# SEAME-pt/Team02-ObjectDetection

Hardware: AMD Instinct MI355X
Metric: images/sec fwd+bwd MobileNetV2UNet 256x512 bs=32/GPU (higher is better)
Workload: dtype f32; 1 GPU; MobileNetV2UNet 10-class fwd+bwd+Adam, 256x512, bs=32/GPU (BASELINE configs[1]); model=MobileNetV2UNet, global_batch=32, parallelism=dp1, collectives=RCCL (torch.distributed nccl), optimizer=seg_amd.Adam (HIP, one launch)

## Files before the change

### include/segamd.h

```cpp
#ifndef SEGAMD_H
#define SEGAMD_H
#include <hip/hip_runtime.h>
#include <stdint.h>
#ifdef __cplusplus
extern "C" {
#endif



int seg_conv_igemm(const float* in, long ldin, int N, int H, int W, int Cin,
                   const float* wk, int ldk, const float* bias,
                   float* out, long ldout, int Ho, int Wo, int Cout,
                   int ks, int stride, int pad,
                   const float* add, long ldadd, float* stat, hipStream_t stream);
int seg_conv_igemm_act(const float* in, long ldin, int N, int H, int W, int Cin,
                       const float* wk, int ldk, const float* bias,
                       float* out, long ldout, int Ho, int Wo, int Cout,
                       int ks, int stride, int pad,
                       const float* add, long ldadd, float* stat, int act, float* work, int splits,
                       hipStream_t stream);
int seg_conv_igemm_bf16(const float* in, long ldin, int N, int H, int W, int Cin,
                        const float* wk, int ldk, const float* bias,
                        float* out, long ldout, int Ho, int Wo, int Cout,
                        int ks, int stride, int pad,
                        const float* add, long ldadd, float* stat, int act, float* work, int splits,
                        hipStream_t stream);
int seg_conv_igemm_f16(const float* in, long ldin, int N, int H, int W, int Cin,
                       const float* wk, int ldk, const float* bias,
                       float* out, long ldout, int Ho, int Wo, int Cout,
                       int ks, int stride, int pad,
                       const float* add, long ldadd, float* stat, int act, float* work, int splits,
                       hipStream_t stream);
int seg_conv_pw_row_tiles(long M);
int seg_conv_pw(const float* in, long ldin, long M, int K, const float* wk, int ldk, const float* bias,
                float* out, long ldout, int N, const float* add, long ldadd, float* stat,
                const float* in_scale, const float* in_shift, int in_act, hipStream_t stream);
int seg_conv_igemm_splits(long M, int Cout, int Cin, int ks);
int seg_conv_igemm_tiles(long M, int Cout);
int seg_conv_igemm_plan_b1(long M, int Cout, int Cin, int ks, int* out);
int seg_conv_igemm_act_ic(const float* in, long ldin, int N, int H, int W, int Cin, const float* wk, int ldk,
                          const float* bias, float* out, long ldout, int Ho, int Wo, int Cout, int ks, int stride,
                          int pad, const float* add, long ldadd, int act, float* work, int splits, int tile, unsigned* cnt,
                          hipStream_t stream);
int seg_conv_igemm_bf16_ic(const float* in, long ldin, int N, int H, int W, int Cin, const float* wk, int ldk,
                           const float* bias, float* out, long ldout, int Ho, int Wo, int Cout, int ks, int stride,
                           int pad, const float* add, long ldadd, int act, float* work, int splits, int tile, unsigned* cnt,
                           hipStream_t stream);
int seg_conv_igemm_f16_ic(const float* in, long ldin, int N, int H, int W, int Cin, const float* wk, int ldk,
                          const float* bias, float* out, long ldout, int Ho, int Wo, int Cout, int ks, int stride,
                          int pad, const float* add, long ldadd, int act, float* work, int splits, int tile, unsigned* cnt,
                          hipStream_t stream);

int seg_conv_igemm_bnout_ok(long M, int Cout, int bf16);
int seg_conv_igemm_bnout(const float* in, long ldin, int N, int H, int W, int Cin, const float* wk, int ldk,
                         float* out, long ldout, int Cout, int ks, const float* add, long ldadd,
                         const float* by, long ldby, const float* bscale, const float* bshift,
                         const float* bmean, int bact, float* bpart, hipStream_t stream);

int seg_igemm_force_tile(int t);
int seg_conv_igemm_tile(long M, int Cout);
int seg_conv_igemm_row_tiles(long M, int Cout, int* tile_rows);

int seg_pack_conv_weight(const float* w, float* wk, int Cout, int Cin, int ks, int ldk,
                         int mode, int kin_pad, hipStream_t stream);

int seg_conv_wgrad_splits(long M, int Cout, int Cin, int ks);
int seg_conv_wgrad_splits_bf16(long M, int Cout, int Cin, int ks);
int seg_conv_wgrad(const float* dy, long lddy, const float* x, long ldx,
                   int N, int H, int W, int Cin, int Ho, int Wo, int Cout,
                   int ks, int stride, int pad, float* part, int splits, hipStream_t stream);

int seg_conv_wgrad_bf16(const float* dy, long lddy, const float* x, long ldx,
                        int N, int H, int W, int Cin, int Ho, int Wo, int Cout,
                        int ks, int stride, int pad, float* part, int splits, hipStream_t stream);

int seg_conv_igemm_xf(const float* in, long ldin, int N, int H, int W, int Cin,
                      const float* wk, int ldk, const float* bias,
                      float* out, long ldout, int Ho, int Wo, int Cout,
                      int ks, int stride, int pad,
                      const float* add, long ldadd, float* stat, const float* in_scale, const float* in_shift,
                      int in_act, hipStream_t stream);
int seg_conv_igemm_bf16_xf(const float* in, long ldin, int N, int H, int W, int Cin,
                           const float* wk, int ldk, const float* bias,
                           float* out, long ldout, int Ho, int Wo, int Cout,
                           int ks, int stride, int pad,
                           const float* add, long ldadd, float* stat, const float* in_scale, const float* in_shift,
                           int in_act, hipStream_t stream);
int seg_conv_wgrad_xf(const float* dy, long lddy, const float* x, long ldx,
                      int N, int H, int W, int Cin, int Ho, int Wo, int Cout,
                      int ks, int stride, int pad, float* part, int splits,
                      const float* in_scale, const float* in_shift, int in_act, hipStream_t stream);
int seg_conv_wgrad_bf16_xf(const float* dy, long lddy, const float* x, long ldx,
                           int N, int H, int W, int Cin, int Ho, int Wo, int Cout,
                           int ks, int stride, int pad, float* part, int splits,
                           const float* in_scale, const float* in_shift, int in_act, hipStream_t stream);

int seg_conv_wgrad_reduce(const float* part, int splits, float* dw, int Cout, int Cin, int ks,
                          int mode, int accumulate, hipStream_t stream);

int seg_conv_wino_pick(int N, int H, int W, int Cin, int Cout);
int seg_conv_wino_tile_rows(void);
int seg_conv_wino_row_tiles(int N, int H, int W);
int seg_conv_wino(const float* in, long ldin, int N, int H, int W, int Cin, const float* wk, int ldk,
                  const float* bias, float* out, long ldout, int Cout, const float* add, long ldadd,
                  float* stat, float* work, hipStream_t stream);
int seg_conv_wino_fused(const float* in, long ldin, int N, int H, int W, int Cin, const float* wk, int ldk,
                        const float* bias, float* out, long ldout, int Cout, const float* add, long ldadd, float* stat,
                        hipStream_t stream);
int seg_conv_wino_fused_ok(int N, int H, int W, long ldin);
int seg_conv_wino_wgrad_pick(int N, int H, int W, int Cin, int Cout);
int seg_conv_wino_wgrad_splits(int N, int H, int W, int Cin, int Cout);
int seg_conv_wino_wgrad(const float* dy, long lddy, const float* x, long ldx, int N, int H, int W, int Cin,
                        int Cout, float* part, int splits, hipStream_t stream);
int seg_conv_wino_wgrad16_splits(int N, int H, int W, int Cin, int Cout);
int seg_conv_wino_wgrad16(const float* dy, long lddy, const float* x, long ldx, int N, int H, int W, int Cin,
                          int Cout, float* part, int splits, hipStream_t stream);
int seg_conv_wino_wgrad_reduce(float* part, int splits, float* dw, int Cout, int Cin, int Cin_pad,
                               int accumulate, hipStream_t stream);

int seg_conv_halo_ok(int N, int H, int W, int Cin, int Cout);
int seg_conv_halo_pick(int N, int H, int W, int Cin, int Cout);
int seg_conv_halo_row_tiles(int N, int H, int W);
int seg_conv_halo(const float* in, long ldin, int N, int H, int W, int Cin, const float* wk, int ldk,
                  const float* bias, float* out, long ldout, int Cout, const float* add, long ldadd,
                  float* stat, hipStream_t stream);

typedef struct seg_pack_job {
  const float* w;
  float* wk;
  int cout, cin, ks, ldk, mode, kin_pad;
  int blk0, nblk;
} seg_pack_job;
int seg_pack_batch(const void* jobs, int njobs, long nblocks, hipStream_t stream);

int seg_pack_dw_weight(const float* w, float* wk, int C, hipStream_t stream);
int seg_dw_fwd(const float* in, long ldin, int N, int H, int W, int C,
               const float* in_scale, const float* in_shift, int in_act, const float* wk,
               float* out, long ldout, int Ho, int Wo, int stride, hipStream_t stream);
int seg_dw_fwd_bias_act(const float* in, long ldin, int N, int H, int W, int C, const float* wk,
                        const float* bias, int act, float* out, long ldout, int Ho, int Wo, int stride,
                        hipStream_t stream);
int seg_dw_dgrad(const float* dy, long lddy, int N, int Ho, int Wo, int C, const float* wk,
// ... 321 lines not shown
```

### team02-objectdetection_amd/csrc/igemm.hip

```cpp
#include "igemm_impl.h"

int seg_igemm_forced_tile = -1;

SEG_API int seg_conv_igemm_act(const float* in, long ldin, int N, int H, int W, int Cin,
                               const float* wk, int ldk, const float* bias,
                               float* out, long ldout, int Ho, int Wo, int Cout,
                               int ks, int stride, int pad,
                               const float* add, long ldadd, float* stat, int act, float* work, int splits,
                               hipStream_t stream) {
  return conv_igemm_impl<float>(in, ldin, N, H, W, Cin, wk, ldk, bias, out, ldout, Ho, Wo, Cout, ks, stride, pad,
                                add, ldadd, stat, act, work, splits, stream);
}

SEG_API int seg_conv_igemm_xf(const float* in, long ldin, int N, int H, int W, int Cin,
                              const float* wk, int ldk, const float* bias,
                              float* out, long ldout, int Ho, int Wo, int Cout,
                              int ks, int stride, int pad,
                              const float* add, long ldadd, float* stat, const float* in_scale, const float* in_shift,
                              int in_act, hipStream_t stream) {
  if (!in_scale) return (int)hipErrorInvalidValue;
  return conv_igemm_impl<float>(in, ldin, N, H, W, Cin, wk, ldk, bias, out, ldout, Ho, Wo, Cout, ks, stride, pad,
                                add, ldadd, stat, SEG_ACT_NONE, nullptr, 1, stream, in_scale, in_shift, in_act);
}

SEG_API int seg_conv_igemm_bnout_ok(long M, int Cout, int bf16) { return igemm_bnout_tile_ok(M, Cout, bf16 ? 2 : 4); }

SEG_API int seg_conv_igemm_bnout(const float* in, long ldin, int N, int H, int W, int Cin, const float* wk, int ldk,
                                 float* out, long ldout, int Cout, int ks, const float* add, long ldadd,
                                 const float* by, long ldby, const float* bscale, const float* bshift,
                                 const float* bmean, int bact, float* bpart, hipStream_t stream) {
  return conv_igemm_impl<float>(in, ldin, N, H, W, Cin, wk, ldk, nullptr, out, ldout, H, W, Cout, ks, 1, ks / 2, add,
                                ldadd, nullptr, SEG_ACT_NONE, nullptr, 1, stream, nullptr, nullptr, 0, by, ldby,
                                bscale, bshift, bmean, bact, bpart);
}

SEG_API int seg_conv_igemm(const float* in, long ldin, int N, int H, int W, int Cin,
                           const float* wk, int ldk, const float* bias,
                           float* out, long ldout, int Ho, int Wo, int Cout,
                           int ks, int stride, int pad,
                           const float* add, long ldadd, float* stat, hipStream_t stream) {
  return seg_conv_igemm_act(in, ldin, N, H, W, Cin, wk, ldk, bias, out, ldout, Ho, Wo, Cout, ks, stride, pad, add,
                            ldadd, stat, SEG_ACT_NONE, nullptr, 1, stream);
}

SEG_API int seg_conv_igemm_act_ic(const float* in, long ldin, int N, int H, int W, int Cin,
                                   const float* wk, int ldk, const float* bias, float* out, long ldout, int Ho, int Wo,
                                   int Cout, int ks, int stride, int pad, const float* add, long ldadd, int act,
                                   float* work, int splits, int tile, unsigned* cnt, hipStream_t stream) {
  return conv_igemm_impl<float>(in, ldin, N, H, W, Cin, wk, ldk, bias, out, ldout, Ho, Wo, Cout, ks, stride, pad, add,
                              ldadd, nullptr, act, work, splits, stream, nullptr, nullptr, 0, (const float*)nullptr, 0, nullptr,
                              nullptr, nullptr, 0, nullptr, cnt, tile);
}

SEG_API int seg_conv_igemm_tiles(long M, int Cout) {
  const int t = pick_tile(M, Cout);
  return (int)(((M + kTiles[t].bm - 1) / kTiles[t].bm) * ((Cout + kTiles[t].bn - 1) / kTiles[t].bn));
}

SEG_API int seg_conv_igemm_plan_b1(long M, int Cout, int Cin, int ks, int* out) {
  if (!out) return (int)hipErrorInvalidValue;
  int splits = 1, tile = -1;
  if (M > 0 && Cout > 0 && Cin > 0 && seg_igemm_forced_tile < 0) {
    const long K = (long)ks * ks * Cin;
    const int t = pick_tile(M, Cout);
    const long blocks = ((M + kTiles[t].bm - 1) / kTiles[t].bm) * ((Cout + kTiles[t].bn - 1) / kTiles[t].bn);
    const int nk = seg_cdiv(K, igemm_bk((int)K));
    if (blocks < 256) {
      if (nk <= 24) {
        tile = 3;
      } else {
        tile = 12;
        const long b12 = ((M + 127) / 128) * ((Cout + 63) / 64);
        long s = std::min<long>(std::min<long>(32, (256 + b12 - 1) / b12), nk / 4);
        s = std::max<long>(s, 1);
        splits = seg_cdiv(nk, seg_cdiv(nk, (int)s));
      }
    }
  }
  const int tt = tile >= 0 ? tile : pick_tile(std::max<long>(M, 1), std::max(Cout, 1));
  out[0] = splits;
  out[1] = tile;
  out[2] = (int)(((M + kTiles[tt].bm - 1) / kTiles[tt].bm) * ((Cout + kTiles[tt].bn - 1) / kTiles[tt].bn));
  return 0;
}

SEG_API int seg_conv_igemm_splits(long M, int Cout, int Cin, int ks) {
  if (M <= 0 || Cout <= 0 || Cin <= 0) return 1;
  return igemm_splits(M, Cout, ks * ks * Cin);
}

SEG_API int seg_igemm_force_tile(int t) {
  if (t < -1 || t >= kNumTiles) return (int)hipErrorInvalidValue;
  seg_igemm_forced_tile = t;
  return 0;
}

SEG_API int seg_conv_igemm_tile(long M, int Cout) { return pick_tile(M, Cout); }

SEG_API int seg_conv_igemm_row_tiles(long M, int Cout, int* tile_rows) {
  const int bm = kTiles[pick_tile(M, Cout)].bm;
  if (tile_rows) *tile_rows = bm;
  return (int)((M + bm - 1) / bm);
}

__global__ void pack_conv_weight_kernel(const float* __restrict__ w, float* __restrict__ wk,
                                        int Cout, int Cin, int taps, int ldk, int mode, int kin_pad) {
  const int rows = mode == 0 ? Cout : Cin;
  const int kin = kin_pad;
  const long total = (long)rows * ldk;
  for (long i = blockIdx.x * (long)blockDim.x + threadIdx.x; i < total; i += (long)gridDim.x * blockDim.x) {
    const int r = (int)(i / ldk), k = (int)(i - (long)r * ldk);
    float v = 0.f;
    if (k < taps * kin) {
      const int tap = k / kin, c = k - tap * kin;
      if (mode == 0) { if (c < Cin) v = w[((long)r * Cin + c) * taps + tap]; }
      else if (c < Cout) v = w[((long)c * Cin + r) * taps + (taps - 1 - tap)];
    }
    wk[i] = v;
  }
}

SEG_API int seg_pack_conv_weight(const float* w, float* wk, int Cout, int Cin, int ks, int ldk, int mode,
                                 int kin_pad, hipStream_t stream) {
  if (kin_pad < (mode == 0 ? Cin : Cout)) return (int)hipErrorInvalidValue;
  if (ldk < ks * ks * kin_pad) return (int)hipErrorInvalidValue;
  const long total = (long)(mode == 0 ? Cout : Cin) * ldk;
  const int grid = (int)std::min<long>(seg_cdiv(total, 256), 4096);
  hipLaunchKernelGGL(pack_conv_weight_kernel, dim3(grid), dim3(256), 0, stream, w, wk, Cout, Cin, ks * ks, ldk, mode, kin_pad);
  SEG_RET_LAST();
}

struct SegPackJob {
  const float* w;
  float* wk;
  int cout, cin, ks, ldk, mode, kin_pad;
  int blk0, nblk;
};
static_assert(sizeof(SegPackJob) == 48, "seg_pack_job ABI");

__global__ __launch_bounds__(256) void pack_batch_kernel(const SegPackJob* __restrict__ jobs, int njobs) {
  int lo = 0, hi = njobs - 1;
  while (lo < hi) {
    const int mid = (lo + hi + 1) >> 1;
    if (jobs[mid].blk0 <= (int)blockIdx.x) lo = mid; else hi = mid - 1;
  }
  const SegPackJob j = jobs[lo];
  const long i = ((long)blockIdx.x - j.blk0) * 256 + threadIdx.x;
  const int taps = j.ks * j.ks;
  if (j.mode == 2) {
    if (i >= 9L * j.cout) return;
    const int tap = (int)(i / j.cout), c = (int)(i - (long)tap * j.cout);
    j.wk[i] = j.w[c * 9 + tap];
    return;
  }
  if (j.mode == 3 || j.mode == 4) {
    const int rows = j.mode == 3 ? j.cout : j.cin;
    if (i >= (long)rows * j.ldk) return;
    const int r = (int)(i / j.ldk), k = (int)(i - (long)r * j.ldk);
    const bool in = k < (j.mode == 3 ? j.cin : j.cout);
    float g[3][3];
#pragma unroll
    for (int y = 0; y < 3; ++y)
#pragma unroll
      for (int x = 0; x < 3; ++x)
        g[y][x] = !in ? 0.f
                      : j.mode == 3 ? j.w[(((long)r * j.cin + k) * 3 + y) * 3 + x]
                                    : j.w[(((long)k * j.cin + r) * 3 + (2 - y)) * 3 + (2 - x)];
    float h[4][3];
#pragma unroll
    for (int x = 0; x < 3; ++x) {
      h[0][x] = g[0][x];
      h[1][x] = 0.5f * (g[0][x] + g[1][x] + g[2][x]);
      h[2][x] = 0.5f * (g[0][x] - g[1][x] + g[2][x]);
      h[3][x] = g[2][x];
    }
    const long plane = (long)rows * j.ldk;
#pragma unroll
    for (int y = 0; y < 4; ++y) {
      const float u[4] = {h[y][0], 0.5f * (h[y][0] + h[y][1] + h[y][2]), 0.5f * (h[y][0] - h[y][1] + h[y][2]),
// ... 29 lines not shown
```

### team02-objectdetection_amd/csrc/igemm_impl.h

```cpp
#pragma once
#include "common.h"

extern int seg_igemm_forced_tile;

namespace {

__device__ __attribute__((aligned(16))) float g_zero4[4];

struct IgemmArgs {
  const void* in; long ldin;
  const void* wk; int ldk;
  const float* bias;
  const void* add; long ldadd;
  void* out; long ldout;
  float* stat;
  int N, H, W, Cin;
  int Ho, Wo, Cout;
  int stride, pad;
  int K, M;
  int kchunk;
  float* part;
  int act;
  const float* xs; const float* xb; int xact;
  const void* by; long ldby; const float* bsc; const float* bsh; const float* bmu; int bact; float* bpart;
  unsigned* kcnt;
  int kspin;
};

#ifndef SEG_IGEMM_DEPTH
#define SEG_IGEMM_DEPTH 1
#endif
#ifndef SEG_IGEMM_STAGES
#define SEG_IGEMM_STAGES 1
#endif
#ifndef SEG_IGEMM_UT
#define SEG_IGEMM_UT 1
#endif
#ifndef SEG_IGEMM_UT2
#define SEG_IGEMM_UT2 1
#endif
#ifndef SEG_IGEMM_BK
#define SEG_IGEMM_BK 32
#endif

template <int BM, int BN, int WM, int WN, int KS, int BK, bool UT, typename OT = float, typename IT = float,
          bool WB = false, bool BO = false>
__global__ __launch_bounds__(64 * (BM / WM) * (BN / WN)) void igemm_conv_kernel(IgemmArgs a) {
  static_assert(!WB || std::is_same<OT, __bf16>::value, "bf16 weights feed bf16 operands");
  const float* wk32 = static_cast<const float*>(a.wk);
  const __bf16* wk16 = static_cast<const __bf16*>(a.wk);
  const IT* __restrict__ in = static_cast<const IT*>(a.in);
  const IT* add = static_cast<const IT*>(a.add);
  IT* out = static_cast<IT*>(a.out);
  const IT* zero4 = reinterpret_cast<const IT*>(g_zero4);
  constexpr int NT = 64 * (BM / WM) * (BN / WN);
  constexpr bool LP = sizeof(OT) == 2;
  constexpr int LDSR = LP ? BK + 8 : BK + 4;
  using lds_t = OT;
  typedef OT ot4 __attribute__((ext_vector_type(4)));
  typedef OT ot8 __attribute__((ext_vector_type(8)));
  constexpr int VB = WB ? 8 : 4;
  constexpr int KQ = BK / VB;
  constexpr int VA = (sizeof(IT) == 2 && UT) ? 8 : 4;
  static_assert(VA == 4 || std::is_same<OT, IT>::value, "raw 16-byte A copies need OT == IT");
  constexpr int KQA = BK / VA;
  constexpr int A_VEC = BM * KQA, B_VEC = BN * KQ;
  constexpr int A_PER = (A_VEC + NT - 1) / NT;
  constexpr int B_PER = (B_VEC + NT - 1) / NT;
  constexpr int MI = WM / 32, NI = WN / 32;
  constexpr int WAVES_N = BN / WN;
  static_assert(NT == 256 || NT == 512, "4 or 8 waves per block");
  static_assert(NT % KQ == 0 && NT % KQA == 0, "uniform kq per thread");
  static_assert(!LP || BK % 16 == 0, "16-bit MFMA steps are 16 deep");
  static_assert(sizeof(lds_t) * BM * LDSR >= 4 * (BM / WM + 1) * BN, "BN-statistics scratch fits in As");

  constexpr int CSR = BN + 4;
  constexpr int AB_BYTES = SEG_IGEMM_STAGES * (BM + BN) * LDSR * (int)sizeof(lds_t);
  constexpr int C_BYTES = WM * CSR * 4;
  __shared__ __attribute__((aligned(16))) char smem[AB_BYTES > C_BYTES ? AB_BYTES : C_BYTES];
  lds_t (*As)[BM * LDSR] = reinterpret_cast<lds_t (*)[BM * LDSR]>(smem);
  lds_t (*Bs)[BN * LDSR] = reinterpret_cast<lds_t (*)[BN * LDSR]>(smem + SEG_IGEMM_STAGES * BM * LDSR * sizeof(lds_t));

  const int tid = threadIdx.x, lane = tid & 63, wave = tid >> 6;
  const int wm0 = (wave / WAVES_N) * WM, wn0 = (wave % WAVES_N) * WN;
  const int tiles_n = (a.Cout + BN - 1) / BN;
  const int lid = xcd_swizzle(blockIdx.x, gridDim.x);
  const int tn = lid % tiles_n, tm = lid / tiles_n;
  const int m0 = tm * BM, n0 = tn * BN;
  const int kbeg = blockIdx.y * a.kchunk;

  long a_base[A_PER];
  int a_hi0[A_PER], a_wi0[A_PER], a_ci[A_PER], a_ky[A_PER], a_kx[A_PER], a_k[A_PER];
  bool a_ok[A_PER];
#pragma unroll
  for (int i = 0; i < A_PER; ++i) {
    const int idx = tid + i * NT;
    const int row = idx / KQA, kq = idx % KQA;
    const int p = m0 + row;
    a_ok[i] = (idx < A_VEC) && (p < a.M);
    const int pp = a_ok[i] ? p : 0;
    a_k[i] = kq * VA + kbeg;
    const int tap = a_k[i] / a.Cin;
    a_ci[i] = a_k[i] - tap * a.Cin;
    a_ky[i] = tap / KS;
    a_kx[i] = tap - a_ky[i] * KS;
    if (KS == 1) {
      a_base[i] = (long)pp * a.ldin;
      a_hi0[i] = a_wi0[i] = 0;
    } else {
      const int hw = a.Ho * a.Wo;
      const int n = pp / hw, rem = pp - n * hw;
      const int ho = rem / a.Wo, wo = rem - ho * a.Wo;
      a_base[i] = (long)n * a.H * a.W;
      a_hi0[i] = ho * a.stride - a.pad;
      a_wi0[i] = wo * a.stride - a.pad;
    }
  }

  long u_aoff[A_PER], u_boff[B_PER];
  unsigned u_mask[A_PER];
  bool u_bok[B_PER];
  const int u_kq4 = (tid % KQ) * VB;
  const int u_kqa = (tid % KQA) * VA;
  const bool XF = a.xs != nullptr;
  int xch = -1;
  unsigned xvm = 0;
  f32x4 xsc[VA / 4], xsh[VA / 4];
  int u_tap = 0, u_ci = 0;
  long u_toff0 = 0, u_toff1 = 0;
// ... 133 lines not shown
                                         xsc[0], xsh[0], a.xact);
            const f32x4 hi = seg_bn_act4(__builtin_convertvector(__builtin_shufflevector(q, q, 4, 5, 6, 7), f32x4),
                                         xsc[VA / 4 - 1], xsh[VA / 4 - 1], a.xact);
            v = __builtin_bit_cast(f32x4, seg_cat8(__builtin_convertvector(lo, bf16x4),
                                                   __builtin_convertvector(hi, bf16x4)));
          } else {
            v = seg_bn_act4(v, xsc[0], xsh[0], a.xact);
            if constexpr (sizeof(IT) == 2) {
              v = __builtin_convertvector(__builtin_convertvector(v, bf16x4), f32x4);
            }
          }
        }
        if constexpr (VA == 8)
          *reinterpret_cast<f32x4*>(&As[buf][(idx / KQA) * LDSR + (idx % KQA) * 8]) = v;
        else
          st_op(&As[buf][(idx / KQA) * LDSR + (idx % KQA) * 4], v);
      }
    }
#pragma unroll
    for (int i = 0; i < B_PER; ++i) {
      const int idx = tid + i * NT;
      if (B_VEC % NT == 0 || idx < B_VEC) {
        if constexpr (WB)
          *reinterpret_cast<f32x4*>(&Bs[buf][(idx / KQ) * LDSR + (idx % KQ) * 8]) = rb[i];
        else
          st_op(&Bs[buf][(idx / KQ) * LDSR + (idx % KQ) * 4], rb[i]);
      }
    }
  };

  f32x16 acc[MI][NI];
#pragma unroll
  for (int mi = 0; mi < MI; ++mi)
#pragma unroll
    for (int ni = 0; ni < NI; ++ni)
#pragma unroll
      for (int r = 0; r < 16; ++r) acc[mi][ni][r] = 0.f;

  const int nk = (min(a.K - kbeg, a.kchunk) + BK - 1) / BK;
  const int lrow = lane & 31, lk = (lane >> 5) * 4;
  auto compute = [&](int cur) {
    if constexpr (LP) {
      const int lk8 = (lane >> 5) * 8;
#pragma unroll
      for (int ks = 0; ks < BK / 16; ++ks) {
        ot8 af[MI], bfr[NI];
#pragma unroll
        for (int mi = 0; mi < MI; ++mi)
          af[mi] = *reinterpret_cast<const ot8*>(&As[cur][(wm0 + mi * 32 + lrow) * LDSR + ks * 16 + lk8]);
#pragma unroll
        for (int ni = 0; ni < NI; ++ni)
          bfr[ni] = *reinterpret_cast<const ot8*>(&Bs[cur][(wn0 + ni * 32 + lrow) * LDSR + ks * 16 + lk8]);
#pragma unroll
        for (int mi = 0; mi < MI; ++mi)
#pragma unroll
          for (int ni = 0; ni < NI; ++ni) {
            if constexpr (std::is_same<OT, _Float16>::value)
              acc[mi][ni] = __builtin_amdgcn_mfma_f32_32x32x16_f16(af[mi], bfr[ni], acc[mi][ni], 0, 0, 0);
            else
              acc[mi][ni] = __builtin_amdgcn_mfma_f32_32x32x16_bf16(af[mi], bfr[ni], acc[mi][ni], 0, 0, 0);
          }
      }
      return;
    }
#pragma unroll
    for (int ks = 0; ks < BK / 8; ++ks) {
      f32x4 af[MI], bf[NI];
#pragma unroll
      for (int mi = 0; mi < MI; ++mi)
        af[mi] = *reinterpret_cast<const f32x4*>(&As[cur][(wm0 + mi * 32 + lrow) * LDSR + ks * 8 + lk]);
#pragma unroll
      for (int ni = 0; ni < NI; ++ni)
        bf[ni] = *reinterpret_cast<const f32x4*>(&Bs[cur][(wn0 + ni * 32 + lrow) * LDSR + ks * 8 + lk]);
#pragma unroll
      for (int kk = 0; kk < 4; ++kk)
#pragma unroll
        for (int mi = 0; mi < MI; ++mi)
#pragma unroll
          for (int ni = 0; ni < NI; ++ni)
            acc[mi][ni] = __builtin_amdgcn_mfma_f32_32x32x2f32(af[mi][kk], bf[ni][kk], acc[mi][ni], 0, 0, 0);
    }
  };

#if SEG_IGEMM_STAGES == 1
  f32x4 ra[A_PER], rb[B_PER];
  load_tiles(kbeg, ra, rb);
  for (int kt = 0; kt < nk; ++kt) {
    store_tiles(0, ra, rb);
    __syncthreads();
    if (kt + 1 < nk) load_tiles(kbeg + (kt + 1) * BK, ra, rb);
    compute(0);
    __syncthreads();
  }
#elif SEG_IGEMM_DEPTH == 1
  f32x4 ra[A_PER], rb[B_PER];
  load_tiles(kbeg, ra, rb);
  store_tiles(0, ra, rb);
  __syncthreads();
  for (int kt = 0; kt < nk; ++kt) {
    const int cur = kt & 1;
    if (kt + 1 < nk) load_tiles(kbeg + (kt + 1) * BK, ra, rb);
    compute(cur);
    if (kt + 1 < nk) store_tiles(cur ^ 1, ra, rb);
    __syncthreads();
  }
#else
  f32x4 ra0[A_PER], rb0[B_PER], ra1[A_PER], rb1[B_PER];
  load_tiles(kbeg, ra0, rb0);
  store_tiles(0, ra0, rb0);
  if (nk > 1) load_tiles(kbeg + BK, ra1, rb1);
  __syncthreads();
  for (int kt = 0; kt < nk; kt += 2) {
    if (kt + 2 < nk) load_tiles(kbeg + (kt + 2) * BK, ra0, rb0);
    compute(0);
    if (kt + 1 < nk) store_tiles(1, ra1, rb1);
    __syncthreads();
    if (kt + 1 >= nk) break;
    if (kt + 3 < nk) load_tiles(kbeg + (kt + 3) * BK, ra1, rb1);
    compute(1);
    if (kt + 2 < nk) store_tiles(0, ra0, rb0);
    __syncthreads();
  }
#endif

  if (a.part) {
    float* P = a.part + (long)blockIdx.y * a.M * a.Cout;
    const bool ic = a.kcnt != nullptr;
#pragma unroll
    for (int ni = 0; ni < NI; ++ni) {
      const int col = n0 + wn0 + ni * 32 + lrow;
      if (col >= a.Cout) continue;
#pragma unroll
      for (int mi = 0; mi < MI; ++mi)
#pragma unroll
        for (int r = 0; r < 16; ++r) {
          const int row = m0 + wm0 + mi * 32 + (r & 3) + 8 * (r >> 2) + 4 * (lane >> 5);
          if (row < a.M) {
            if (ic) seg_st_wt(P + (long)row * a.Cout + col, acc[mi][ni][r]);
            else P[(long)row * a.Cout + col] = acc[mi][ni][r];
          }
        }
    }
    if (!ic) return;
    const int S = gridDim.y, z = blockIdx.y;
    auto piece = [&](int pz) {
      constexpr int E = BM * BN;
      const int e0 = (int)((long)pz * E / S), e1 = (int)((long)(pz + 1) * E / S);
      const long total = (long)a.M * a.Cout;
      for (int e = e0 + tid; e < e1; e += NT) {
        const int r = e / BN, c = e - r * BN, row = m0 + r, col = n0 + c;
        if (row >= a.M || col >= a.Cout) continue;
        const long i = (long)row * a.Cout + col;
        float v = 0.f;
        for (int z0 = 0; z0 < S; z0 += 16) {
          float q[16];
#pragma unroll
          for (int j = 0; j < 16; ++j) q[j] = z0 + j < S ? seg_ld_wt(a.part + (z0 + j) * total + i) : 0.f;
#pragma unroll
          for (int j = 0; j < 16; ++j)
            if (z0 + j < S) v += q[j];
        }
        if (a.bias) v += a.bias[col];
        if (add) v += (float)add[(long)row * a.ldadd + col];
        if (a.act) v = seg_act(v, a.act);
        out[(long)row * a.ldout + col] = static_cast<IT>(v);
      }
    };
    seg_tile_combine(a.kcnt + 4 * lid, S, z, a.kspin, reinterpret_cast<int*>(smem), piece);
    return;
  }
  float bcol[NI];
#pragma unroll
  for (int ni = 0; ni < NI; ++ni) {
    const int col = n0 + wn0 + ni * 32 + lrow;
    bcol[ni] = (a.bias && col < a.Cout) ? a.bias[col] : 0.f;
#pragma unroll
    for (int mi = 0; mi < MI; ++mi)
#pragma unroll
      for (int r = 0; r < 16; ++r) acc[mi][ni][r] += bcol[ni];
  }
  if (a.stat) {
    constexpr int WR = BM / WM;
    float* red = reinterpret_cast<float*>(&As[0][0]);
    float* tmean = red + WR * BN;
    const int nrows = min(BM, a.M - m0);
    const int wr = wave / WAVES_N;
#pragma unroll
    for (int pass = 0; pass < 2; ++pass) {
#pragma unroll
      for (int ni = 0; ni < NI; ++ni) {
        const int cl = wn0 + ni * 32 + lrow;
        const float mu = pass ? tmean[cl] : 0.f;
        float s = 0.f;
#pragma unroll
        for (int mi = 0; mi < MI; ++mi)
#pragma unroll
          for (int r = 0; r < 16; ++r) {
            const int row = m0 + wm0 + mi * 32 + (r & 3) + 8 * (r >> 2) + 4 * (lane >> 5);
            const float d = acc[mi][ni][r] - mu;
            s += row < a.M ? (pass ? d * d : d) : 0.f;
          }
        s += __shfl_xor(s, 32, 64);
        if (lane < 32) red[wr * BN + cl] = s;
      }
      __syncthreads();
      if (tid < BN) {
// ... 84 lines not shown
            }
          }
        } else {
#pragma unroll
          for (int j = 0; j < VO; ++j) {
            if (col + j >= a.Cout) break;
            float x = o[j];
            if (ad) x += (float)ad[j];
            if (a.act) x = seg_act(x, a.act);
            const IT q = static_cast<IT>(x);
            dst[j] = q;
            if constexpr (bon) bacc(j, (float)q, (float)by[(long)row * a.ldby + col + j]);
          }
        }
    };
    constexpr int NVB = (WM * VPR + NT - 1) / NT;
    f32x4 yreg[BOK ? BM / WM : 1][BOK ? NVB : 1];
    if constexpr (BOK) {
#pragma unroll
      for (int b = 0; b < BM / WM; ++b)
#pragma unroll
        for (int k = 0; k < NVB; ++k) {
          const int v = tid + k * NT, rr = v / VPR, cv = (v - rr * VPR) * VO;
          const int row = m0 + b * WM + rr, col = n0 + cv;
          const bool ok = v < WM * VPR && row < a.M && col + VO <= a.Cout;
          yreg[b][k] = *reinterpret_cast<const f32x4*>(ok ? (const void*)(by + (long)row * a.ldby + col)
                                                          : (const void*)g_zero4);
        }
    }
#pragma unroll
    for (int b = 0; b < BM / WM; ++b) {
      __syncthreads();
      if (wm0 == b * WM) {
#pragma unroll
        for (int ni = 0; ni < NI; ++ni)
#pragma unroll
          for (int mi = 0; mi < MI; ++mi)
#pragma unroll
            for (int r = 0; r < 16; ++r)
              Cs[(mi * 32 + (r & 3) + 8 * (r >> 2) + 4 * (lane >> 5)) * CSR + wn0 + ni * 32 + lrow] = acc[mi][ni][r];
      }
      __syncthreads();
      if constexpr (BOK) {
#pragma unroll
        for (int k = 0; k < NVB; ++k) {
          const int v = tid + k * NT;
          if (v < WM * VPR) store_vec(b, v, yreg[b][k]);
        }
      } else {
        for (int v = tid; v < WM * VPR; v += NT) store_vec(b, v, f32x4{});
      }
    }
    if constexpr (BOK) {
      {
        constexpr int NW = NT / 64;
        float* red = reinterpret_cast<float*>(smem);
#pragma unroll
        for (int j = 0; j < VO; ++j) {
#pragma unroll
          for (int o = VPR; o < 64; o *= 2) {
            bs0[j] += __shfl_xor(bs0[j], o, 64);
            bs1[j] += __shfl_xor(bs1[j], o, 64);
          }
        }
        __syncthreads();
        if (lane < VPR) {
#pragma unroll
          for (int j = 0; j < VO; ++j) {
            red[(0 * NW + wave) * BN + bcv + j] = bs0[j];
            red[(1 * NW + wave) * BN + bcv + j] = bs1[j];
          }
        }
        __syncthreads();
        for (int q = tid; q < 2 * BN; q += NT) {
          const int h = q / BN, c = q - h * BN;
          float t = 0.f;
#pragma unroll
          for (int k = 0; k < NW; ++k) t += red[(h * NW + k) * BN + c];
          if (n0 + c < a.Cout) a.bpart[((long)tm * 2 + h) * a.Cout + n0 + c] = t;
        }
      }
    }
  }
}

thread_local bool g_igemm_ic_used = false;

template <int BM, int BN, int WM, int WN, int BK, typename OT, typename IT, bool WB = false>
int launch_igemm_bk(IgemmArgs a, int ks, hipStream_t s) {
  const int grid = seg_cdiv(a.M, BM) * seg_cdiv(a.Cout, BN);
  const int splits = seg_cdiv(a.K, a.kchunk);
  const bool ut = SEG_IGEMM_UT && (SEG_IGEMM_UT2 ? a.Cin >= BK : a.Cin % BK == 0) &&
                  (sizeof(IT) == 4 || (a.Cin % 8 == 0 && a.ldin % 8 == 0));
  constexpr int NT = 64 * (BM / WM) * (BN / WN);
  if (a.xs && !ut) return (int)hipErrorInvalidValue;
  if (a.kcnt) {
    int occ = 0;
    const void* fn = ks == 1 ? (ut ? (const void*)igemm_conv_kernel<BM, BN, WM, WN, 1, BK, true, OT, IT, WB, false>
                                   : (const void*)igemm_conv_kernel<BM, BN, WM, WN, 1, BK, false, OT, IT, WB, false>)
                             : (ut ? (const void*)igemm_conv_kernel<BM, BN, WM, WN, 3, BK, true, OT, IT, WB, false>
                                   : (const void*)igemm_conv_kernel<BM, BN, WM, WN, 3, BK, false, OT, IT, WB, false>);
    if (hipOccupancyMaxActiveBlocksPerMultiprocessor(&occ, fn, NT, 0) != hipSuccess ||
        (long)grid * splits > (long)occ * seg_num_cus() || splits > 32) {
      (void)hipGetLastError();
      a.kcnt = nullptr;
    }
  }
  g_igemm_ic_used = a.kcnt != nullptr;
#define SEG_IG(KS, U, B) hipLaunchKernelGGL((igemm_conv_kernel<BM, BN, WM, WN, KS, BK, U, OT, IT, WB, B>), dim3(grid, splits), dim3(NT), 0, s, a)
  constexpr int VPR = BN / (16 / (int)sizeof(IT));
  if constexpr (std::is_same<OT, IT>::value && BN % (16 / (int)sizeof(IT)) == 0 && 64 % VPR == 0) {
    if (a.bpart) {
      if (ks == 1) {
        if (ut) SEG_IG(1, true, true); else SEG_IG(1, false, true);
      } else {
        if (ut) SEG_IG(3, true, true); else SEG_IG(3, false, true);
      }
      SEG_RET_LAST();
    }
  }
  if (a.bpart) return (int)hipErrorInvalidValue;
  if (ks == 1) {
    if (ut) SEG_IG(1, true, false); else SEG_IG(1, false, false);
  } else {
    if (ut) SEG_IG(3, true, false); else SEG_IG(3, false, false);
  }
#undef SEG_IG
  SEG_RET_LAST();
}

inline int igemm_bk(int K) { return (SEG_IGEMM_BK != 16 && (K <= 64 || (K % SEG_IGEMM_BK != 0 && K < 512))) ? 16 : SEG_IGEMM_BK; }

template <int BM, int BN, int WM, int WN, typename OT = float, typename IT = float, bool WB = false>
int launch_igemm(IgemmArgs a, int ks, int splits, hipStream_t s) {
  int bk = igemm_bk(a.K);
  if (sizeof(OT) == 2 && bk == SEG_IGEMM_BK && a.Cin >= 64 && a.K >= 256 && splits == 1) bk = 64;
  const int nk = seg_cdiv(a.K, bk);
  a.kchunk = seg_cdiv(nk, splits) * bk;
  if constexpr (sizeof(OT) == 2) {
    if (bk == 64) return launch_igemm_bk<BM, BN, WM, WN, 64, OT, IT, WB>(a, ks, s);
  }
  if (bk == 16) return launch_igemm_bk<BM, BN, WM, WN, 16, OT, IT, WB>(a, ks, s);
  return launch_igemm_bk<BM, BN, WM, WN, SEG_IGEMM_BK, OT, IT, WB>(a, ks, s);
}

struct TileCfg {
  int bm, bn, wm, wn;
  float eff;
};
constexpr TileCfg kTiles[] = {
    {128, 128, 64, 64, 1.00f}, {64, 128, 32, 64, 0.95f}, {128, 64, 64, 32, 0.95f}, {64, 64, 32, 32, 0.85f},
    {128, 96, 32, 96, 0.97f},  {128, 160, 32, 160, 0.95f}, {256, 32, 64, 32, 0.90f}, {128, 32, 32, 32, 0.92f},
    {128, 128, 64, 32, 0.0f}, {128, 128, 32, 64, 0.0f}, {256, 128, 64, 64, 0.0f}, {128, 256, 64, 64, 0.0f},
    {128, 64, 32, 32, 0.0f}, {256, 64, 64, 32, 0.0f}, {64, 128, 32, 32, 0.0f},
};

constexpr int kNumTiles = (int)(sizeof(kTiles) / sizeof(kTiles[0]));

int pick_tile(long M, int N);
inline bool igemm_bnout_tile_ok(long M, int N, int es) {
  const int bn = kTiles[pick_tile(M, N)].bn, vo = 16 / es;
  return bn % vo == 0 && 64 % (bn / vo) == 0;
}

int pick_tile(long M, int N) {
  if (seg_igemm_forced_tile >= 0) return seg_igemm_forced_tile;
  int best = 0;
  double best_score = -1.0;
  for (int i = 0; i < (int)(sizeof(kTiles) / sizeof(kTiles[0])); ++i) {
    const TileCfg& t = kTiles[i];
    const long bm_tiles = (M + t.bm - 1) / t.bm, bn_tiles = (N + t.bn - 1) / t.bn;
    const long blocks = bm_tiles * bn_tiles;
    const double util = (double)M * N / ((double)bm_tiles * t.bm * bn_tiles * t.bn);
    const double fill = std::min(1.0, (double)blocks / 512.0);
    const double score = util * t.eff * fill;
    if (score > best_score + 1e-9) {
      best_score = score;
      best = i;
    }
  }
  return best;
}



int igemm_splits(long M, int Cout, int K) {
  const int t = pick_tile(M, Cout);
  const long blocks = ((M + kTiles[t].bm - 1) / kTiles[t].bm) * ((Cout + kTiles[t].bn - 1) / kTiles[t].bn);
  const int nk = seg_cdiv(K, igemm_bk(K));
  if (blocks >= 256 || nk < 8) return 1;
  int s = (int)std::min<long>(seg_cdiv(512, blocks), nk / 4);
  s = std::min(s, 64);
  if (s < 2) return 1;
// ... 83 lines not shown
```

### team02-objectdetection_amd/seg_amd/_lib.py

```python
from __future__ import annotations

import ctypes
import os
import threading

from .build import LIB_PATH, source_hash

_V = ctypes.c_void_p
_I = ctypes.c_int
_L = ctypes.c_long
_F = ctypes.c_float

PROTOTYPES = {
    "seg_conv_igemm": (_I, [_V, _L, _I, _I, _I, _I, _V, _I, _V, _V, _L, _I, _I, _I, _I, _I, _I, _V, _L, _V, _V]),
    "seg_conv_igemm_act": (_I, [_V, _L, _I, _I, _I, _I, _V, _I, _V, _V, _L, _I, _I, _I, _I, _I, _I, _V, _L, _V, _I,
                                _V, _I, _V]),
    "seg_conv_igemm_bf16": (_I, [_V, _L, _I, _I, _I, _I, _V, _I, _V, _V, _L, _I, _I, _I, _I, _I, _I, _V, _L, _V, _I,
                                 _V, _I, _V]),
    "seg_conv_igemm_f16": (_I, [_V, _L, _I, _I, _I, _I, _V, _I, _V, _V, _L, _I, _I, _I, _I, _I, _I, _V, _L, _V, _I,
                                _V, _I, _V]),
    "seg_conv_igemm_splits": (_I, [_L, _I, _I, _I]),
    "seg_igemm_force_tile": (_I, [_I]),
    "seg_conv_igemm_tile": (_I, [_L, _I]),
    "seg_conv_halo_ok": (_I, [_I, _I, _I, _I, _I]),
    "seg_conv_halo_pick": (_I, [_I, _I, _I, _I, _I]),
    "seg_conv_halo_row_tiles": (_I, [_I, _I, _I]),
    "seg_conv_halo": (_I, [_V, _L, _I, _I, _I, _I, _V, _I, _V, _V, _L, _I, _V, _L, _V, _V]),
    "seg_conv_wino_pick": (_I, [_I, _I, _I, _I, _I]),
    "seg_conv_wino_row_tiles": (_I, [_I, _I, _I]),
    "seg_conv_wino_tile_rows": (_I, []),
    "seg_conv_wino": (_I, [_V, _L, _I, _I, _I, _I, _V, _I, _V, _V, _L, _I, _V, _L, _V, _V, _V]),
    "seg_conv_wino_fused": (_I, [_V, _L, _I, _I, _I, _I, _V, _I, _V, _V, _L, _I, _V, _L, _V, _V]),
    "seg_conv_wino_fused_ok": (_I, [_I, _I, _I, _L]),
    "seg_conv_wino_wgrad_pick": (_I, [_I, _I, _I, _I, _I]),
    "seg_conv_wino_wgrad_splits": (_I, [_I, _I, _I, _I, _I]),
    "seg_conv_wino_wgrad": (_I, [_V, _L, _V, _L, _I, _I, _I, _I, _I, _V, _I, _V]),
    "seg_conv_wino_wgrad16_splits": (_I, [_I, _I, _I, _I, _I]),
    "seg_conv_wino_wgrad16": (_I, [_V, _L, _V, _L, _I, _I, _I, _I, _I, _V, _I, _V]),
    "seg_conv_wino_wgrad_reduce": (_I, [_V, _I, _V, _I, _I, _I, _I, _V]),
    "seg_pack_batch": (_I, [_V, _I, _L, _V]),
    "seg_conv_igemm_row_tiles": (_I, [_L, _I, _V]),
    "seg_pack_conv_weight": (_I, [_V, _V, _I, _I, _I, _I, _I, _I, _V]),
    "seg_conv_wgrad_splits": (_I, [_L, _I, _I, _I]),
    "seg_conv_wgrad_splits_bf16": (_I, [_L, _I, _I, _I]),
    "seg_conv_wgrad": (_I, [_V, _L, _V, _L, _I, _I, _I, _I, _I, _I, _I, _I, _I, _I, _V, _I, _V]),
    "seg_conv_wgrad_bf16": (_I, [_V, _L, _V, _L, _I, _I, _I, _I, _I, _I, _I, _I, _I, _I, _V, _I, _V]),
    "seg_conv_wgrad_reduce": (_I, [_V, _I, _V, _I, _I, _I, _I, _I, _V]),
    "seg_pack_dw_weight": (_I, [_V, _V, _I, _V]),
    "seg_dw_fwd": (_I, [_V, _L, _I, _I, _I, _I, _V, _V, _I, _V, _V, _L, _I, _I, _I, _V]),
    "seg_dw_fwd_bias_act": (_I, [_V, _L, _I, _I, _I, _I, _V, _V, _I, _V, _L, _I, _I, _I, _V]),
    "seg_dw_dgrad": (_I, [_V, _L, _I, _I, _I, _I, _V, _V, _L, _I, _I, _I, _I, _V]),
    "seg_dw_wgrad_blocks": (_L, [_I, _I, _I, _I]),
    "seg_dw_wgrad": (_I, [_V, _L, _V, _L, _I, _I, _I, _I, _V, _V, _I, _I, _I, _I, _V, _V]),
    "seg_nchw_to_nhwc": (_I, [_V, _I, _I, _I, _I, _V, _I, _V]),
    "seg_chan_workspace_floats": (_L, [_L, _I]),
    "seg_bn_stats": (_I, [_V, _L, _L, _I, _V, _V, _F, _F, _V, _V, _V, _V, _V, _V, _V, _V, _V]),
    "seg_bn_stats_tiles": (_I, [_V, _I, _I, _L, _I, _V, _V, _F, _F, _V, _V, _V, _V, _V, _V, _V, _V]),
    "seg_bn_stats_tiles_ws": (_I, [_V, _I, _I, _L, _I, _V, _V, _F, _F, _V, _V, _V, _V, _V, _V, _V, _V, _V]),
    "seg_bn_stats_tiles_work_floats": (_L, [_I, _I]),
    "seg_bn_eval_coef": (_I, [_V, _V, _V, _V, _F, _I, _V, _V, _V]),
    "seg_bn_apply": (_I, [_V, _L, _L, _I, _V, _V, _I, _V, _L, _V, _L, _V]),
    "seg_bn_backward": (_I, [_V, _L, _V, _L, _L, _I, _V, _V, _V, _V, _V, _I, _V, _V, _V, _V, _L, _V]),
    "seg_bn_eval_backward": (_I, [_V, _L, _V, _L, _L, _I, _V, _V, _I, _V, _L, _V]),
    "seg_bn_frozen_backward": (_I, [_V, _L, _V, _L, _L, _I, _V, _V, _V, _V, _F, _I, _V, _V, _V, _V, _L, _V]),
    "seg_colsum": (_I, [_V, _L, _L, _I, _V, _V, _I, _V]),
    "seg_add": (_I, [_V, _L, _V, _L, _L, _I, _V, _L, _V]),
    "seg_upsample_fwd": (_I, [_V, _L, _I, _I, _I, _I, _V, _L, _I, _I, _I, _V]),
    "seg_upsample_bwd": (_I, [_V, _L, _I, _I, _I, _I, _I, _V, _L, _I, _I, _I, _I, _V]),
    "seg_upsample_to_nchw": (_I, [_V, _L, _I, _I, _I, _I, _V, _I, _I, _I, _V]),
    "seg_maxpool2_fwd": (_I, [_V, _L, _I, _I, _I, _I, _V, _L, _V]),
    "seg_maxpool2_bwd": (_I, [_V, _L, _V, _L, _I, _I, _I, _I, _V, _L, _I, _V]),
    "seg_ce_workspace_floats": (_L, [_L]),
    "seg_ce_upsample_loss": (_I, [_V, _L, _I, _I, _I, _I, _V, _I, _I, _I, _V, _V, _V]),
    "seg_ce_upsample_grad": (_I, [_V, _L, _I, _I, _I, _I, _V, _I, _I, _I, _V, _V, _V, _L, _V]),
    "seg_ce_upsample_eval": (_I, [_V, _L, _I, _I, _I, _I, _V, _I, _I, _I, _V, _V, _V, _V]),
    "seg_cew_workspace_floats": (_L, [_L]),
    "seg_cew_upsample_loss": (_I, [_V, _L, _I, _I, _I, _I, _V, _I, _I, _I, _V, _F, _I, _V, _V, _V]),
    "seg_cew_upsample_grad": (_I, [_V, _L, _I, _I, _I, _I, _V, _I, _I, _I, _V, _F, _V, _V, _V, _L, _V]),
    "seg_cew_upsample_eval": (_I, [_V, _L, _I, _I, _I, _I, _V, _I, _I, _I, _V, _F, _I, _V, _V, _V, _V]),
    "seg_sl_workspace_floats": (_L, [_L]),
    "seg_sl_upsample_loss": (_I, [_V, _L, _I, _I, _I, _I, _V, _I, _I, _I, _V, _F, _F, _F, _F, _F, _V, _V, _V, _V]),
    "seg_sl_upsample_eval": (_I, [_V, _L, _I, _I, _I, _I, _V, _I, _I, _I, _V, _F, _F, _F, _F, _F, _V, _V, _V, _V,
                                  _V]),
    "seg_sl_upsample_grad": (_I, [_V, _L, _I, _I, _I, _I, _V, _I, _I, _I, _V, _F, _F, _F, _F, _V, _V, _V, _V, _L,
                                  _V]),
    "seg_bn_fold_batch": (_I, [_V, _I, _L, _V]),
    "seg_preprocess_bgr": (_I, [_V, _I, _I, _I, _L, _V, _I, _I, _I, _F, _F, _F, _F, _F, _F, _V]),
    "seg_argmax_nearest": (_I, [_V, _L, _I, _I, _I, _I, _I, _I, _V, _I, _I, _V]),
    "seg_resize_u8": (_I, [_V, _I, _I, _I, _L, _V, _I, _I, _I, _V, _V]),
    "seg_augment": (_I, [_V, _V, _I, _I, _I, _V, _F, _F, _F, _F, _F, _F, _V, _V, _V]),
    "seg_adam_step": (_I, [_V, _V, _I, _I, _F, _F, _F, _F, _V]),
    "seg_adam_step_skip": (_I, [_V, _V, _I, _I, _F, _F, _F, _F, _V, _V]),
    "seg_adamw_step": (_I, [_V, _V, _I, _I, _F, _F, _F, _F, _V, _V, _V]),
    "seg_grad_norm_workspace_floats": (_L, [_I]),
    "seg_grad_sumsq": (_I, [_V, _V, _I, _I, _F, _V, _V, _V]),
    "seg_grad_scale": (_I, [_V, _V, _I, _I, _V, _V]),
    "seg_tape_fn_index": (_I, [ctypes.c_char_p]),
    "seg_tape_fn_nargs": (_I, [_I]),
    "seg_tape_create": (_I, [_V, _I, _V, _L, _I, _V]),
    "seg_tape_destroy": (_I, [_V]),
    "seg_tape_set_arg": (_I, [_V, _L, _L]),
    "seg_tape_timing": (_I, [_V, _V, _I, _I]),
    "seg_tape_elapsed": (_I, [_V, _V]),
    "seg_tape_timeline": (_I, [_V, _I, _V]),
    "seg_tape_run": (_I, [_V, _I, _V, _V, _V]),
    "seg_set_combine_spin": (_I, [_I]),
# ... 116 lines not shown
```

### team02-objectdetection_amd/seg_amd/engine.py

```python
from __future__ import annotations

import contextlib
import ctypes
import os
from typing import NamedTuple

import torch
from torch import nn

from ._lib import call, query as _query

_PURE_QUERIES = {"seg_chan_workspace_floats", "seg_conv_wgrad_splits", "seg_conv_wgrad_splits_bf16", "seg_dw_wgrad_blocks",
                 "seg_conv_igemm_splits", "seg_ce_workspace_floats", "seg_conv_wino_row_tiles", "seg_conv_wino_tile_rows",
                 "seg_conv_halo_row_tiles", "seg_conv_wino_wgrad_splits", "seg_conv_wino_wgrad16_splits",
                 "seg_mbconv_ok"}
_QCACHE = {}


def query(name, *args):
    if name not in _PURE_QUERIES:
        return _query(name, *args)
    key = (name, args)
    r = _QCACHE.get(key)
    if r is None:
        r = _QCACHE[key] = _query(name, *args)
    return r
from .mobilenet import ConvBNReLU6, InvertedResidual

ACT_NONE, ACT_RELU, ACT_RELU6 = 0, 1, 2
IGNORE_INDEX = -100
_ROW_TILES = {}


_IG2 = {}
_TILE_GEN = 0


class Route(NamedTuple):
    family: str
    name: str
    timer: str | None
    mode: int | None = None
    ldk: int = 0
    tiles: tuple | None = None
    work: int = 0
    zero: bool = False
    splits: int = 0
    bnout: str | None = None
    fallback: "Route | None" = None


def _pw_pick(op, v: int):
    if not PW or op.kind != "igemm" or op.ks != 1 or op.stride != 1:
        return False, False
    i, y = op.inp, op.y
    if y.M < PW_MIN_ROWS:
        return False, False
    rows = lambda *ts: all(t.ld % v == 0 and t.off % v == 0 for t in ts)
    fwd = 8 <= op.cin_pad <= 32 and op.cin_pad % 8 == 0 and op.cout <= 192 and rows(i, y)
    kin = r4(op.cout)
    bwd = not op.first and 8 <= kin <= 32 and kin % 8 == 0 and op.cin <= 192 and rows(i) and kin % v == 0
    return fwd, bwd


def igemm2_plan(M: int, cout: int, cin: int, ks: int):
    key = (M, cout, cin, ks)
    if key not in _IG2:
        out = (ctypes.c_long * 4)()
        ok = query("seg_conv_igemm2_plan", M, cout, cin, ks, ctypes.addressof(out))
        _IG2[key] = tuple(out) if ok else None
    return _IG2[key]


def force_tiles(igemm: int | None = None, igemm2: int | None = None) -> None:
    global _TILE_GEN
    _TILE_GEN += 1
    if igemm is not None:
        _query("seg_igemm_force_tile", int(igemm))
    if igemm2 is not None:
        _query("seg_igemm2_force_tile", int(igemm2))
    _ROW_TILES.clear()
    _IG2.clear()
    _QCACHE.clear()


def r8(c: int) -> int:
    return (c + 7) & ~7


def r4(c: int) -> int:
    return (c + 3) & ~3


class KernelTimer:

    def __init__(self, kinds=None, max_replays=64):
        self.records = []
        self.kinds = kinds
        self.tapes = []
        self.max_replays = max_replays

        self.collected = []

    def collect(self, tape):
        if tape in self.tapes:
            torch.cuda.synchronize()
            self.collected += tape.elapsed()
            self.tapes.remove(tape)

    def elapsed(self):
        out = [(k, f, a.elapsed_time(b) * 1e-3) for k, f, a, b in self.records] + self.collected
        for t in self.tapes:
            out += t.elapsed()
        return out


TIMER: KernelTimer | None = None

def _stat_ptrs(st, C):
    b = st.data_ptr()
    return b, b + 4 * C, b + 8 * C, b + 12 * C


def _timed_call(kind, flops, name, *args):
    if TIMER is None or (TIMER.kinds is not None and kind not in TIMER.kinds):
        return call(name, *args)
    a = torch.cuda.Event(enable_timing=True)
    b = torch.cuda.Event(enable_timing=True)
    a.record()
    call(name, *args)
    b.record()
    TIMER.records.append((kind, flops, a, b))


class Act:
    __slots__ = ("buf", "off", "ld", "C", "N", "H", "W")

    def __init__(self, buf, off, ld, C, N, H, W):
        self.buf, self.off, self.ld, self.C, self.N, self.H, self.W = buf, off, ld, C, N, H, W

    @property
    def M(self):
        return self.N * self.H * self.W

    def key(self):
        return (self.buf, self.off, self.C)

    def slice(self, off, C):
        return Act(self.buf, self.off + off, self.ld, C, self.N, self.H, self.W)



IMAGE = "image"


class ConvOp:

    def __init__(self, kind, conv: nn.Conv2d, bn, act, inp, out, y, res, xform=None):
        self.kind, self.conv, self.bn, self.act = kind, conv, bn, act
        self.inp, self.out, self.y, self.res = inp, out, y, res
        self.lazy = False
        self.xform = xform
        self.route_f = self.route_d = self.route_w = None
# ... 1603 lines not shown
```

Before: 2035 images/s.

## Add register-streaming fp32 1x1 igemm path that bypasses LDS tiling

Adds a streaming variant of the 1x1 fp32 implicit-GEMM conv kernel. Each wave loads its A and B fragments directly from global memory into a register ring and feeds MFMA without LDS staging. The fused BN/activation input transform is applied in registers using coefficients cached in shared memory. It is selected only for specific tiles when the block count fits within the CU count and K>=384, targeting latency-bound small-grid layers. In exchange it adds register pressure, a new code path, and a force-override knob.

```diff
diff --git a/include/segamd.h b/include/segamd.h
--- a/include/segamd.h
+++ b/include/segamd.h
@@ -58,6 +58,8 @@
                          const float* bmean, int bact, float* bpart, hipStream_t stream);
 
 int seg_igemm_force_tile(int t);
+int seg_igemm_force_stream(int mode);
+int seg_conv_igemm_streams(long M, int Cout, int K, int ks);
 int seg_conv_igemm_tile(long M, int Cout);
 int seg_conv_igemm_row_tiles(long M, int Cout, int* tile_rows);
 
diff --git a/team02-objectdetection_amd/csrc/igemm.hip b/team02-objectdetection_amd/csrc/igemm.hip
--- a/team02-objectdetection_amd/csrc/igemm.hip
+++ b/team02-objectdetection_amd/csrc/igemm.hip
@@ -1,6 +1,10 @@
 #include "igemm_impl.h"
 
 int seg_igemm_forced_tile = -1;
+int seg_igemm_forced_stream = -1;
+
+constexpr int kStreamMinK = 384;
+bool seg_igemm_stream_rule(long blocks, int K, bool xf) { return xf && blocks <= seg_num_cus() && K >= kStreamMinK; }
 
 SEG_API int seg_conv_igemm_act(const float* in, long ldin, int N, int H, int W, int Cin,
                                const float* wk, int ldk, const float* bias,
@@ -95,6 +99,18 @@
   return 0;
 }
 
+SEG_API int seg_igemm_force_stream(int mode) {
+  if (mode < -1 || mode > 1) return (int)hipErrorInvalidValue;
+  seg_igemm_forced_stream = mode;
+  return 0;
+}
+
+SEG_API int seg_conv_igemm_streams(long M, int Cout, int K, int ks) {
+  if (M <= 0 || Cout <= 0 || K <= 0) return 0;
+  const TileCfg& t = kTiles[pick_tile(M, Cout)];
+  return igemm_stream_ok(t.bm, t.bn, t.wm, t.wn, igemm_bk(K), M, Cout, K, ks, true) ? 1 : 0;
+}
+
 SEG_API int seg_conv_igemm_tile(long M, int Cout) { return pick_tile(M, Cout); }
 
 SEG_API int seg_conv_igemm_row_tiles(long M, int Cout, int* tile_rows) {
diff --git a/team02-objectdetection_amd/csrc/igemm_impl.h b/team02-objectdetection_amd/csrc/igemm_impl.h
--- a/team02-objectdetection_amd/csrc/igemm_impl.h
+++ b/team02-objectdetection_amd/csrc/igemm_impl.h
@@ -2,6 +2,8 @@
 #include "common.h"
 
 extern int seg_igemm_forced_tile;
+extern int seg_igemm_forced_stream;
+bool seg_igemm_stream_rule(long blocks, int K, bool xf);
 
 namespace {
 
@@ -43,8 +45,13 @@
 #define SEG_IGEMM_BK 32
 #endif
 
+#ifndef SEG_IGEMM_STREAM_VGPRS
+#define SEG_IGEMM_STREAM_VGPRS 64
+#endif
+constexpr int igemm_stream_steps(int ni) { return SEG_IGEMM_STREAM_VGPRS / (4 * (1 + ni)); }
+
 template <int BM, int BN, int WM, int WN, int KS, int BK, bool UT, typename OT = float, typename IT = float,
-          bool WB = false, bool BO = false>
+          bool WB = false, bool BO = false, bool ST = false>
 __global__ __launch_bounds__(64 * (BM / WM) * (BN / WN)) void igemm_conv_kernel(IgemmArgs a) {
   static_assert(!WB || std::is_same<OT, __bf16>::value, "bf16 weights feed bf16 operands");
   const float* wk32 = static_cast<const float*>(a.wk);
@@ -344,6 +351,88 @@
     }
   };
 
+  if constexpr (ST) {
+    static_assert(KS == 1 && UT && !LP && !WB && std::is_same<IT, float>::value, "streaming: fp32 1x1 only");
+    static_assert(WM == 32 && BN == WN && BM / WM == NT / 64, "streaming: each wave owns its rows alone");
+    constexpr int SD = igemm_stream_steps(NI);
+    const int S = nk * (BK / 8);
+    const int KF = a.K / 8;
+    const float* ap = in + (long)min(m0 + wm0 + lrow, a.M - 1) * a.ldin + lk;
+    const float* bp[NI];
+#pragma unroll
+    for (int ni = 0; ni < NI; ++ni) bp[ni] = wk32 + (long)min(n0 + wn0 + ni * 32 + lrow, a.Cout - 1) * a.ldk + lk;
+    float* xl = reinterpret_cast<float*>(smem);
+    if (XF) {
+      for (int i = tid * 4; i < 8 * S; i += NT * 4) {
+        *reinterpret_cast<f32x4*>(xl + i) = ld4(i < a.K ? a.xs + i : g_zero4);
+        *reinterpret_cast<f32x4*>(xl + 8 * S + i) = ld4(i < a.K ? a.xb + i : g_zero4);
+      }
+      __syncthreads();
+    }
+    auto ldstep = [&](int s, f32x4& ra, f32x4 (&rb)[NI]) {
+      const intptr_t kin = -(intptr_t)(8 * s + lk < a.K), z = (intptr_t)g_zero4;
+      ra = ld4(reinterpret_cast<const float*>(z + (((intptr_t)(ap + 8 * s) - z) & kin)));
+#pragma unroll
+      for (int ni = 0; ni < NI; ++ni)
+        rb[ni] = ld4(reinterpret_cast<const float*>(z + (((intptr_t)(bp[ni] + 8 * s) - z) & kin)));
+    };
+    auto coef = [&](int s, f32x4& cs, f32x4& cb) {
+      const int o = 8 * min(s, S - 1) + lk;
+      cs = *reinterpret_cast<const f32x4*>(xl + o);
+      cb = *reinterpret_cast<const f32x4*>(xl + 8 * S + o);
+    };
+    auto run = [&](auto xf) {
+      constexpr bool X = decltype(xf)::value;
+      f32x4 ra[SD], rb[SD][NI];
+      f32x4 af = {0.f, 0.f, 0.f, 0.f}, c1s = af, c1b = af;
+      auto round = [&](int s0, auto fast_t, auto tail_t) {
+        constexpr bool FAST = decltype(fast_t)::value, TAIL = decltype(tail_t)::value;
+#pragma unroll
+        for (int j = 0; j < SD; ++j) {
+          const int s = s0 + j;
+          if (TAIL && s >= S) break;
+          f32x4 c2s, c2b;
+          if constexpr (X) coef(s + 2, c2s, c2b);
+          const f32x4 a4 = X ? af : ra[j];
+#pragma unroll
+          for (int kk = 0; kk < 4; ++kk)
+#pragma unroll
+            for (int ni = 0; ni < NI; ++ni)
+              acc[0][ni] = __builtin_amdgcn_mfma_f32_32x32x2f32(a4[kk], rb[j][ni][kk], acc[0][ni], 0, 0, 0);
+          if constexpr (X) {
+            af = seg_bn_act4(ra[(j + 1) % SD], c1s, c1b, a.xact);
+            c1s = c2s;
+            c1b = c2b;
+          }
+          if constexpr (FAST) {
+            ra[j] = ld4(ap + 8 * (s + SD));
+#pragma unroll
+            for (int ni = 0; ni < NI; ++ni) rb[j][ni] = ld4(bp[ni] + 8 * (s + SD));
+          } else if constexpr (!TAIL) {
+            ldstep(s + SD, ra[j], rb[j]);
+          }
+          __builtin_amdgcn_sched_barrier(0);
+        }
+      };
+#pragma unroll
+      for (int j = 0; j < SD; ++j) ldstep(j, ra[j], rb[j]);
+      if constexpr (X) {
+        coef(0, c1s, c1b);
+        af = seg_bn_act4(ra[0], c1s, c1b, a.xact);
+        coef(1, c1s, c1b);
+      }
+      int s0 = 0;
+      for (; s0 + 2 * SD <= KF; s0 += SD) round(s0, std::true_type{}, std::false_type{});
+      for (; s0 + SD <= S; s0 += SD) round(s0, std::false_type{}, std::false_type{});
+      round(s0, std::false_type{}, std::true_type{});
+    };
+    if (XF) {
+      run(std::true_type{});
+      __syncthreads();
+    } else {
+      run(std::false_type{});
+    }
+  } else {
 #if SEG_IGEMM_STAGES == 1
   f32x4 ra[A_PER], rb[B_PER];
   load_tiles(kbeg, ra, rb);
@@ -384,6 +473,7 @@
     __syncthreads();
   }
 #endif
+  }
 
   if (a.part) {
     float* P = a.part + (long)blockIdx.y * a.M * a.Cout;
@@ -634,6 +724,20 @@
       }
     }
   }
+}
+
+constexpr bool igemm_stream_tile(int bm, int bn, int wm, int wn) {
+  return bm == 128 && wm == 32 && bn == wn && (bn == 32 || bn == 96);
+}
+
+inline bool igemm_stream_ok(int bm, int bn, int wm, int wn, int bk, long M, int Cout, int K, int ks, bool xf) {
+  const long lds = std::max<long>((long)SEG_IGEMM_STAGES * (bm + bn) * (bk + 4) * 4, (long)wm * (bn + 4) * 4);
+  if (!igemm_stream_tile(bm, bn, wm, wn) || ks != 1 || seg_igemm_forced_stream == 0 || M <= 0 || Cout <= 0 || K <= 0 ||
+      8L * ((K + bk - 1) / bk) * bk > lds)
+    return false;
+  if (seg_igemm_forced_stream == 1) return true;
+  const long blocks = ((M + bm - 1) / bm) * ((Cout + bn - 1) / bn);
+  return seg_igemm_stream_rule(blocks, K, xf);
 }
 
 thread_local bool g_igemm_ic_used = false;
@@ -661,6 +765,21 @@
   g_igemm_ic_used = a.kcnt != nullptr;
 #define SEG_IG(KS, U, B) hipLaunchKernelGGL((igemm_conv_kernel<BM, BN, WM, WN, KS, BK, U, OT, IT, WB, B>), dim3(grid, splits), dim3(NT), 0, s, a)
   constexpr int VPR = BN / (16 / (int)sizeof(IT));
+  if constexpr (std::is_same<OT, float>::value && std::is_same<IT, float>::value && !WB &&
+                igemm_stream_tile(BM, BN, WM, WN)) {
+    if (splits == 1 && !a.part && igemm_stream_ok(BM, BN, WM, WN, BK, a.M, a.Cout, a.K, ks, a.xs != nullptr)) {
+#define SEG_IGS(B) hipLaunchKernelGGL((igemm_conv_kernel<BM, BN, WM, WN, 1, BK, true, float, float, false, B, true>), dim3(grid, 1), dim3(NT), 0, s, a)
+      if (!a.bpart) {
+        SEG_IGS(false);
+        SEG_RET_LAST();
+      }
+      if constexpr (64 % VPR == 0) {
+        SEG_IGS(true);
+        SEG_RET_LAST();
+      }
+#undef SEG_IGS
+    }
+  }
   if constexpr (std::is_same<OT, IT>::value && BN % (16 / (int)sizeof(IT)) == 0 && 64 % VPR == 0) {
     if (a.bpart) {
       if (ks == 1) {
diff --git a/team02-objectdetection_amd/seg_amd/_lib.py b/team02-objectdetection_amd/seg_amd/_lib.py
--- a/team02-objectdetection_amd/seg_amd/_lib.py
+++ b/team02-objectdetection_amd/seg_amd/_lib.py
@@ -22,6 +22,8 @@
     "seg_conv_igemm_splits": (_I, [_L, _I, _I, _I]),
     "seg_igemm_force_tile": (_I, [_I]),
     "seg_conv_igemm_tile": (_I, [_L, _I]),
+    "seg_igemm_force_stream": (_I, [_I]),
+    "seg_conv_igemm_streams": (_I, [_L, _I, _I, _I]),
     "seg_conv_halo_ok": (_I, [_I, _I, _I, _I, _I]),
     "seg_conv_halo_pick": (_I, [_I, _I, _I, _I, _I]),
     "seg_conv_halo_row_tiles": (_I, [_I, _I, _I]),
diff --git a/team02-objectdetection_amd/seg_amd/engine.py b/team02-objectdetection_amd/seg_amd/engine.py
--- a/team02-objectdetection_amd/seg_amd/engine.py
+++ b/team02-objectdetection_amd/seg_amd/engine.py
@@ -72,13 +72,15 @@
     return _IG2[key]
 
 
-def force_tiles(igemm: int | None = None, igemm2: int | None = None) -> None:
+def force_tiles(igemm: int | None = None, igemm2: int | None = None, stream: int | None = None) -> None:
     global _TILE_GEN
     _TILE_GEN += 1
     if igemm is not None:
         _query("seg_igemm_force_tile", int(igemm))
     if igemm2 is not None:
         _query("seg_igemm2_force_tile", int(igemm2))
+    if stream is not None:
+        _query("seg_igemm_force_stream", int(stream))
     _ROW_TILES.clear()
     _IG2.clear()
     _QCACHE.clear()
```

Result: no change. 2035 images/s (-0.0%).
